# coecms/xmhw

Hardware: AMD Instinct MI355X
Metric: grid-cells/sec for threshold() on 40yr daily SST (higher is better)
Workload: dtype f32 in / f64 out; 1 GPU; 0.25deg global (configs[2]): 1036800 cells per step, 1982-2021 (T=14610), windowHalfWidth=5, pctile=90, smoothPercentileWidth=31, nan_frac=0.0, skipna=False; cells_rank0=1036800, T=14610, D=366, kernel=clim_sorted_f32 (sorted row-lists in LDS, 2 lanes per cell, layout 40), slabs=1, gather=none

## Files before the change

xmhw_amd/csrc/capi.cpp:

```cpp
#include "../../include/xmhw_amd.h"

#include <hip/hip_runtime.h>
#include <unistd.h>

#include <cerrno>

#include <algorithm>
#include <cstdio>
#include <cstdlib>
#include <atomic>
#include <cstring>
#include <map>
#include <memory>
#include <mutex>
#include <new>
#include <string>
#include <type_traits>
#include <vector>

#include "kernels.h"
#include "plan.h"

namespace {

// ... 1081 lines not shown
    const int32_t y2 = v2 >= 0 ? xmhw::ring2_pick_yps(plan->host.w, plan->host.ntracks, v2) : 0;
    *layout = (ring && y2 > 0 && xmhw::ring2_f32_supported(plan->host.w, y2, v2)) ? v2 : -1;
    return XMHW_OK;
}
int xmhw_plan_set_ring2(xmhw_plan* plan, int32_t variant) { return xmhw_plan_set_layout(plan, variant); }
int xmhw_plan_ring2_in_use(const xmhw_plan* plan, int32_t* variant) { return xmhw_plan_layout_in_use(plan, variant); }
int xmhw_plan_f64_mode(const xmhw_plan* plan, int32_t* variant) {
    if (!plan || !variant) return fail(XMHW_ERR_INVALID, "NULL argument");
    *variant = resolve_kernel(plan, 8) == XMHW_KERNEL_RING ? x64_choice(plan).variant : -1;
    return XMHW_OK;
}
int xmhw_plan_destroy(xmhw_plan* plan) {
    delete plan;
    return XMHW_OK;
}
int xmhw_plan_info(const xmhw_plan* plan, int32_t* D, int32_t* ntracks, int32_t* kernel, int32_t* nsteps,
                   int32_t* step_min) {
    if (!plan) return fail(XMHW_ERR_INVALID, "plan is NULL");
    if (D) *D = plan->host.D;
    if (ntracks) *ntracks = plan->host.ntracks;
    if (kernel) *kernel = resolve_kernel(plan, 4);
    if (nsteps) *nsteps = plan->host.nsteps;
    if (step_min) *step_min = plan->host.step_min;
    return XMHW_OK;
}
int xmhw_plan_doys(const xmhw_plan* plan, int32_t* doys_out) {
    if (!plan || !doys_out) return fail(XMHW_ERR_INVALID, "NULL argument");
    std::memcpy(doys_out, plan->host.doys.data(), sizeof(int32_t) * plan->host.doys.size());
    return XMHW_OK;
}
int xmhw_plan_set_kernel(xmhw_plan* plan, int32_t kernel) {
    if (!plan) return fail(XMHW_ERR_INVALID, "plan is NULL");
    if (kernel < XMHW_KERNEL_AUTO || kernel > XMHW_KERNEL_GENERIC)
        return fail(XMHW_ERR_INVALID, "unknown kernel selector");
    plan->host.kernel_choice = kernel;
    return XMHW_OK;
}
int xmhw_plan_set_timing(xmhw_plan* plan, int32_t enable) {
    if (!plan) return fail(XMHW_ERR_INVALID, "plan is NULL");
    plan->timing = enable != 0;
    return XMHW_OK;
}
int xmhw_plan_kernel_ms(xmhw_plan* plan, int32_t calls_back, float* ms) {
    if (!plan || !ms) return fail(XMHW_ERR_INVALID, "NULL argument");
    if (calls_back < 0 || calls_back >= 16 || static_cast<uint64_t>(calls_back) >= plan->tcalls)
        return fail(XMHW_ERR_INVALID, "no such timed call");
    const int slot = static_cast<int>((plan->tcalls - 1 - static_cast<uint64_t>(calls_back)) % 16);
    if (!plan->tev[2 * slot] || !plan->tev[2 * slot + 1]) return fail(XMHW_ERR_INVALID, "no such timed call");
    HIP_TRY(hipEventSynchronize(plan->tev[2 * slot + 1]));
    HIP_TRY(hipEventElapsedTime(ms, plan->tev[2 * slot], plan->tev[2 * slot + 1]));
    return XMHW_OK;
}
int xmhw_plan_set_narrowing(xmhw_plan* plan, int32_t enable) {
    if (!plan) return fail(XMHW_ERR_INVALID, "plan is NULL");
    plan->narrowing = enable != 0;
    return XMHW_OK;
}
int xmhw_plan_narrowed(xmhw_plan* plan, int32_t* narrowed_out) {
    if (!plan || !narrowed_out) return fail(XMHW_ERR_INVALID, "NULL argument");
    *narrowed_out = 0;
    if (!plan->d_narrow_flag) return XMHW_OK;
    uint32_t flag = 1;
    HIP_TRY(hipMemcpy(&flag, plan->d_narrow_flag, sizeof(uint32_t), hipMemcpyDeviceToHost));
    *narrowed_out = flag == 0 ? 1 : 0;
    return XMHW_OK;
}
int xmhw_plan_set_chunks(xmhw_plan* plan, int32_t nchunks) {
    if (!plan) return fail(XMHW_ERR_INVALID, "plan is NULL");
    if (nchunks < 0) return fail(XMHW_ERR_INVALID, "nchunks must be >= 0");
    plan->host.nchunks_req = nchunks;
    return XMHW_OK;
}
int xmhw_plan_chunks_in_use(const xmhw_plan* plan, int64_t C, int32_t* nchunks) {
    if (!plan || !nchunks) return fail(XMHW_ERR_INVALID, "NULL argument");
    if (C < 0) return fail(XMHW_ERR_INVALID, "bad C");
    *nchunks = auto_chunks(plan, std::max<int64_t>(C, 1));
    return XMHW_OK;
}
int xmhw_debug_stats_available(void) { return xmhw::ring_stats_built() ? 1 : 0; }
int xmhw_plan_debug_stats_n(xmhw_plan* plan, int enable, uint64_t* out, int32_t n) {
    if (!plan) return fail(XMHW_ERR_INVALID, "plan is NULL");
    if (out && n <= 0) return fail(XMHW_ERR_INVALID, "n must be > 0");
    if (enable && !plan->d_stats) {
        HIP_TRY(hipMalloc(&plan->d_stats, 16 * sizeof(unsigned long long)));
        HIP_TRY(hipMemset(plan->d_stats, 0, 16 * sizeof(unsigned long long)));
    }
    if (out) {
        if (!plan->d_stats) return fail(XMHW_ERR_INVALID, "stats not enabled");
        unsigned long long all[16];
        HIP_TRY(hipDeviceSynchronize());
        HIP_TRY(hipMemcpy(all, plan->d_stats, sizeof(all), hipMemcpyDeviceToHost));
        HIP_TRY(hipMemset(plan->d_stats, 0, sizeof(all)));
        for (int32_t i = 0; i < std::min<int32_t>(n, 16); ++i) out[i] = all[i];
    }
    return XMHW_OK;
}
int xmhw_plan_debug_stats(xmhw_plan* plan, int enable, uint64_t* out8) {
    return xmhw_plan_debug_stats_n(plan, enable, out8, 8);
}
int xmhw_plan_table(const xmhw_plan* plan, int32_t years_per_lane, uint32_t* table_out,
                    int32_t* ntracks_padded) {
    if (!plan) return fail(XMHW_ERR_INVALID, "plan is NULL");
    if (years_per_lane <= 0) return fail(XMHW_ERR_INVALID, "years_per_lane must be > 0");
    if (plan->host.ntracks > kSubs * years_per_lane)
        return fail(XMHW_ERR_INVALID, "years_per_lane too small for the number of tracks");
    if (ntracks_padded) *ntracks_padded = kSubs * years_per_lane;
    if (table_out) {
        std::vector<uint32_t> tab = plan->host.ring_table(kSubs, years_per_lane);
        std::memcpy(table_out, tab.data(), sizeof(uint32_t) * tab.size());
    }
    return XMHW_OK;
}

int xmhw_plan_sorted_info(const xmhw_plan* plan, int64_t C, int32_t* keys_per_list, int32_t* lds_bytes_per_wave,
                          int32_t* pieces) {
    if (!plan) return fail(XMHW_ERR_INVALID, "plan is NULL");
    const int32_t k = xmhw::sorted_pick_k(plan->host.w, plan->host.ntracks);
    if (k == 0) return fail(XMHW_ERR_UNSUPPORTED, "the sorted-list kernel is not instantiated for this window / record length");
    if (keys_per_list) *keys_per_list = k;
    if (lds_bytes_per_wave) *lds_bytes_per_wave = xmhw::sorted_lds_bytes(plan->host.w, plan->host.ntracks);
    if (pieces) {
        const int64_t waves = (std::max<int64_t>(C, 1) + 31) / 32;
        *pieces = static_cast<int32_t>(plan->host.nchunks_req > 0 ? plan->host.nchunks_req : (1536 + waves - 1) / waves);
    }
    return XMHW_OK;
}

int xmhw_plan_sorted_table(const xmhw_plan* plan, int32_t pieces, int32_t* nchunks, int32_t* nrows, int32_t* ntp,
                           int32_t* chunks_out, uint32_t* table_out, uint32_t* flags_out) {
    if (!plan) return fail(XMHW_ERR_INVALID, "plan is NULL");
    const int32_t yps = xmhw::sorted_pick_yps(plan->host.w, plan->host.ntracks);
    if (yps == 0) return fail(XMHW_ERR_UNSUPPORTED, "the sorted-list kernel is not instantiated for this window / record length");
    const xmhw::Plan::SortedPlan sp = plan->host.sorted_plan(2 * yps, 24, std::max(pieces, 1));
    if (nchunks) *nchunks = static_cast<int32_t>(sp.chunks.size());
    if (nrows) *nrows = static_cast<int32_t>(sp.flags.size());
    if (ntp) *ntp = 2 * yps;
    if (chunks_out)
        for (size_t i = 0; i < sp.chunks.size(); ++i) {
            chunks_out[4 * i + 0] = sp.chunks[i].warm_start;
            chunks_out[4 * i + 1] = sp.chunks[i].begin;
            chunks_out[4 * i + 2] = sp.chunks[i].end;
            chunks_out[4 * i + 3] = sp.chunks[i].trow0;
        }
    if (table_out) std::memcpy(table_out, sp.table.data(), sizeof(uint32_t) * sp.table.size());
    if (flags_out) std::memcpy(flags_out, sp.flags.data(), sizeof(uint32_t) * sp.flags.size());
    return XMHW_OK;
}

int xmhw_clim_raw_f32(xmhw_plan* plan, const float* ts, int64_t C, int64_t ld, double q, int negate,
                      double* thresh, double* seas, int64_t ldo, void* stream) {
    return clim_raw<float>(plan, ts, C, ld, q, negate, thresh, seas, ldo, stream);
}
int xmhw_clim_raw_f64(xmhw_plan* plan, const double* ts, int64_t C, int64_t ld, double q, int negate,
                      double* thresh, double* seas, int64_t ldo, void* stream) {
    return clim_raw<double>(plan, ts, C, ld, q, negate, thresh, seas, ldo, stream);
}

int xmhw_clim_raw_i16(xmhw_plan* plan, const int16_t* codes, int64_t C, int64_t ld, int big_endian, int has_scale,
                      double scale_factor, double add_offset, int has_fill, int32_t fill_code, int decoded_itemsize, double q,
                      int negate, double* thresh, double* seas, int64_t ldo, void* stream) {
    if (!plan) return fail(XMHW_ERR_INVALID, "plan is NULL");
    if (C < 0 || ld < C || ldo < C) return fail(XMHW_ERR_INVALID, "bad C/ld/ldo");
    if (!(q >= 0.0 && q <= 1.0)) return fail(XMHW_ERR_INVALID, "quantile must be in [0, 1]");
    if (decoded_itemsize != 4 && decoded_itemsize != 8) return fail(XMHW_ERR_INVALID, "decoded_itemsize must be 4 or 8");
    if (has_scale && !(scale_factor == scale_factor && add_offset == add_offset && scale_factor != 0.0))
        return fail(XMHW_ERR_INVALID, "scale_factor must be a non-zero number, add_offset a number");
    if (C == 0) return XMHW_OK;
    if (!codes || !thresh || !seas) return fail(XMHW_ERR_INVALID, "NULL device buffer");
    int rc = upload(plan, C);
    if (rc != XMHW_OK) return rc;
    if (!(plan->nchunks_s > 0 && sorted_serves(q)))
        return fail(XMHW_ERR_UNSUPPORTED, "packed input runs on the sorted-list kernel only (w = 5, 9..48 tracks, quantile >= 0.85 or <= 0.15): "
                                         "decode the series (xmhw_decode) and call xmhw_clim_raw_f32 / _f64");
    xmhw::PackedI16 pk;
    pk.swap = big_endian ? 1 : 0;
    pk.fill = has_fill ? fill_code : 0x7FFFFFFF;
// ... 301 lines not shown
```

xmhw_amd/csrc/kernels_sorted.hip:

```cpp
#include <type_traits>

#include "device_common.h"
#include "kernels.h"
#include "packed_src.h"
#include "plan.h"
#include "sortnet_gen.h"

namespace xmhw {
namespace {

typedef __attribute__((address_space(3))) uint32_t lds_u32;
__device__ __forceinline__ uint32_t lds_ld(uint32_t a) { return *reinterpret_cast<lds_u32*>(static_cast<uintptr_t>(a)); }
__device__ __forceinline__ void lds_st(uint32_t a, uint32_t v) { *reinterpret_cast<lds_u32*>(static_cast<uintptr_t>(a)) = v; }

constexpr int kSwap1 = 0xB1;
__device__ __forceinline__ uint32_t swp(uint32_t v) {
    return static_cast<uint32_t>(__builtin_amdgcn_update_dpp(0, static_cast<int>(v), kSwap1, 0xF, 0xF, true));
}
__device__ __forceinline__ double swp(double v) {
    const uint64_t b = static_cast<uint64_t>(__double_as_longlong(v));
    const uint32_t lo = swp(static_cast<uint32_t>(b)), hi = swp(static_cast<uint32_t>(b >> 32));
    return __longlong_as_double(static_cast<long long>((static_cast<uint64_t>(hi) << 32) | lo));
}
__device__ __forceinline__ uint32_t med3u(uint32_t a, uint32_t b, uint32_t c) {
// ... 197 lines not shown
    const char* col = static_cast<const char*>(ts) + (cell_ok ? cell : C - 1) * static_cast<int64_t>(ES);
    const bool mirror = q < 0.5;
    const int kneg = (negate != 0) != mirror ? 1 : 0;
    const uint32_t tmax = static_cast<uint32_t>(Tn - 1);
    const bool padded_last = (YPS - 1) * 2 + sub >= ntracks;
    const uint32_t padmask = padded_last ? 0xFFFFFFFFu : 0u;
    const uint32_t* tab = table + sub;

    const uint32_t lds0 = static_cast<uint32_t>(reinterpret_cast<uintptr_t>((lds_u32*)lds));
    if (lds0 != 0u) __builtin_trap();
    const uint32_t lcell = static_cast<uint32_t>(cw) * 4u;
    for (int i = lane; i < LDS_BYTES / 4; i += 64) lds[i] = 0u;
    __builtin_amdgcn_s_waitcnt(0);
    __builtin_amdgcn_wave_barrier();

    uint32_t P[NL];
    V32 TV = 0;
#define XMHW_RSLO(j) TV[2 * (j)]
#define XMHW_RSHI(j) TV[2 * (j) + 1]
#define XMHW_EX(e, j) TV[12 + 6 * (e) + (j)]
#define XMHW_NVL(j) TV[24 + (j)]
    uint32_t lbase[NL];
#pragma unroll
    for (int j = 0; j < NL; ++j) {
        const int g = sub * NL + j;
        lbase[j] = g < R ? lcell + static_cast<uint32_t>(g) * LSTRIDE : 0x40000000u + lcell;
        P[j] = 0;
    }
    static_assert(KL >= 5, "a list holds a window");
    static_assert(NL == 6 && EXT <= 2, "the register vector holds five values of six lists");
#ifdef XMHW_WARM_SELECT
    uint32_t Ctop = 0, n = 0, B = 0u;
#else
    uint32_t Ctop = 0, n = 0, B = 0xFFFFFFFFu;
#endif
    double total = 0.0;

    const uint32_t ld4 = static_cast<uint32_t>(ld) * ES;
    const char* ap[YPS];
    auto entries_of = [&](int32_t step, uint32_t (&e)[YPS]) {
        const uint32_t* p = tab + static_cast<int64_t>(step - step_min) * NTP;
#pragma unroll
        for (int y = 0; y < YPS; ++y) e[y] = p[y * 2];
    };
    auto point_at = [&](int32_t step) {
        uint32_t e[YPS];
        entries_of(step, e);
#pragma unroll
        for (int y = 0; y < YPS; ++y) {
            const uint32_t t = umin((e[y] >> 1) - 2u, tmax);
            ap[y] = col + static_cast<uint64_t>(t) * ld4;
        }
    };
    auto advance = [&]() {
#pragma unroll
        for (int y = 0; y < YPS; ++y) ap[y] += (y == YPS - 1 && padded_last) ? 0u : ld4;
    };
    typename std::conditional<PACKED, int32_t, float>::type x_in[YPS];
    auto request = [&]() {
#pragma unroll
        for (int y = 0; y < YPS; ++y) {
            if constexpr (PACKED) x_in[y] = static_cast<int32_t>(*reinterpret_cast<const int16_t*>(ap[y]));
            else x_in[y] = *reinterpret_cast<const float*>(ap[y]);
        }
    };
    point_at(ch.warm_start);
    request();

    unsigned long long tacc[8] = {0, 0, 0, 0, 0, 0, 0, 0};
    unsigned long long tlast = 0;
    if constexpr (STATS) tlast = __builtin_amdgcn_s_memtime();
    auto tick = [&](int idx) {
        if constexpr (STATS) {
            __builtin_amdgcn_sched_barrier(0);
            asm volatile("s_waitcnt lgkmcnt(0)" ::: "memory");
            const unsigned long long now = __builtin_amdgcn_s_memtime();
            tacc[idx] += now - tlast;
            tlast = now;
            __builtin_amdgcn_sched_barrier(0);
        }
    };
    uint32_t st_rows = 0, st_iter = 0, st_flag = 0, st_steps = 0;
    uint32_t st_serial = 0, st_ext = 0;
    uint32_t st_more[4] = {0, 0, 0, 0};

    uint32_t e_alo = 0, e_ahi = 0, e_n = 0;
    double e_total = 0.0, e_g = 0.0;

    int32_t ep_s = -1;
    uint32_t ep_eph = 0;
    auto finish_rows = [&]() {
        double th = make_nan(), se = make_nan();
        if (e_n > 0) {
            double v_lo = static_cast<double>(key_f32(e_alo));
            double v_hi = static_cast<double>(key_f32(e_ahi));
            if (mirror) {
                v_lo = -v_lo;
                v_hi = -v_hi;
            }
            se = e_total / static_cast<double>(e_n);
            if constexpr (PACKED) {
                v_lo = packed_value(pk, v_lo);
                v_hi = packed_value(pk, v_hi);
                se = packed_value(pk, se);
            }
            th = numpy_lerp(v_lo, v_hi, e_g);
        }
        if (static_cast<uint32_t>(sub) <= ep_eph && cell_ok) {
            const int64_t row = static_cast<int64_t>(ep_s) - static_cast<int64_t>(ep_eph) + sub;
            thresh[row * ldo + cell] = th;
            seas[row * ldo + cell] = se;
        }
        ep_s = -1;
    };
    bool nan_mode = false;
    uint32_t vi_n = 0xFFFFFFFFu, vi_lo = 0;
    double vi_g = 0.0;
    int m = ((ch.warm_start % R) + R) % R;
    uint32_t sf_cur = __builtin_amdgcn_readfirstlane(sflags[ch.warm_start - step_min]);
    uint32_t sf_nxt = ch.warm_start + 1 < ch.end ? __builtin_amdgcn_readfirstlane(sflags[ch.warm_start + 1 - step_min]) : 0u;
#ifdef XMHW_LOOP_ALIGN
    asm volatile(".p2align " XMHW_STR(XMHW_LOOP_ALIGN) "\n\t.rept " XMHW_STR(XMHW_LOOP_PAD) "\n\ts_nop 0\n\t.endr" ::: "memory");
#endif
    for (int32_t s = ch.warm_start; s < ch.end; ++s) {
        const uint32_t sf = sf_cur;
        const uint32_t sf_nn = s + 2 < ch.end ? sflags[s + 2 - step_min] : 0u;
        uint32_t k[HE];
        double din = 0.0;
        uint32_t nvin = 0;
        float xv[YPS];
        bool packed_fill = false;
        if constexpr (STATS) {
            asm volatile("s_waitcnt vmcnt(0)" ::: "memory");
            tick(5);
        }
        if constexpr (PACKED) {
            if (pk.swap) {
#pragma unroll
                for (int y = 0; y < YPS; ++y)
                    x_in[y] = static_cast<int32_t>(static_cast<int16_t>(__builtin_bswap16(static_cast<uint16_t>(x_in[y]))));
            }
#pragma unroll
            for (int y = 0; y < YPS; ++y) xv[y] = static_cast<float>(x_in[y]);
            if (pk.mode == 1) {
#pragma unroll
                for (int y = 0; y < YPS; ++y) {
                    float f = xv[y] * pk.sf;
                    f = f + pk.of;
                    xv[y] = f;
                }
            }
            bool anyfill = false;
#pragma unroll
            for (int y = 0; y < YPS; ++y) anyfill = anyfill || x_in[y] == pk.fill;
            packed_fill = wave_any(anyfill);
            if (packed_fill) {
#pragma unroll
                for (int y = 0; y < YPS; ++y) xv[y] = x_in[y] == pk.fill ? __uint_as_float(0x7FC00000u) : xv[y];
            }
        } else {
#pragma unroll
            for (int y = 0; y < YPS; ++y) xv[y] = x_in[y];
        }
        bool slow = !(sf & 1u) || nan_mode;
        if (!slow) {
            auto plain_row = [&](auto negc, auto sumc) {
// ... 439 lines not shown
                    pv[j] = sat ? c_ : 0u;
                    need += pv[j];
                }
                need += swp(need);
                if constexpr (STATS) ++st_ext;
                const bool fix = need != 0u;
                auto heads = [&](uint32_t (&hd)[NL]) -> uint32_t {
                    uint32_t lv[NL];
#pragma unroll
                    for (int j = 0; j < NL; ++j) lv[j] = lds_ld(lbase[j] + (P[j] - 1u) * RSTRIDE);
                    uint32_t hm = 0xFFFFFFFFu;
#pragma unroll
                    for (int j = 0; j < NL; ++j) {
                        uint32_t ev = XMHW_EX(0, j);
#pragma unroll
                        for (int e_ = 1; e_ < EXT; ++e_) ev = pv[j] > static_cast<uint32_t>(e_) ? XMHW_EX(e_, j) : ev;
                        hd[j] = (pv[j] != 0u ? ev : lv[j]) - 1u;
                        hm = umin(hm, hd[j]);
                    }
                    return hm;
                };
                uint32_t vlast = a_lo;
                while (wave_any(need != 0u)) {
                    uint32_t hd[NL];
                    const uint32_t hm = heads(hd);
                    const uint32_t ho = swp(hm);
                    const uint32_t cmin = umin(hm, ho);
                    const bool act = need != 0u;
                    const bool win = act && hm == cmin && (sub == 0 || ho != cmin);
                    bool found = false;
#pragma unroll
                    for (int j = 0; j < NL; ++j) {
                        const bool sel = win && !found && hd[j] == cmin;
                        const bool reg = pv[j] != 0u;
                        P[j] = (sel && !reg) ? P[j] - 1u : P[j];
                        pv[j] = (sel && reg) ? pv[j] - 1u : pv[j];
                        found = found || sel;
                    }
                    if (act) {
                        vlast = cmin + 1u;
                        need -= 1u;
                    }
                }
                uint32_t hd[NL];
                uint32_t hm = heads(hd);
                hm = umin(hm, swp(hm)) + 1u;
                uint32_t pvs = 0;
#pragma unroll
                for (int j = 0; j < NL; ++j) pvs += pv[j];
                pvs += swp(pvs);
                if (fix) {
                    a_lo = vlast;
                    a_hi = hm;
                    if (!need2) {
                        if (mirror) a_lo = a_hi;
                        else a_hi = a_lo;
                    }
                    Ctop = Cs - pvs;
#pragma unroll
                    for (int j = 0; j < NL; ++j) flag = flag || (pv[j] == static_cast<uint32_t>(EXT) && XMHW_NVL(j) > static_cast<uint32_t>(K));
                }
            }
        } else {
            uint32_t atb = 0;
#pragma unroll
            for (int j = 0; j < NL; ++j)
                atb |= (P[j] == static_cast<uint32_t>(K) && XMHW_NVL(j) > static_cast<uint32_t>(K)) ? (1u << j) : 0u;
            if (XMHW_COLD(wave_any(atb != 0u))) {
#pragma unroll
                for (int j = 0; j < NL; ++j) {
                    const uint32_t Uj = lds_ld(lbase[j] + static_cast<uint32_t>(K - 1) * RSTRIDE);
                    flag = flag || (((atb >> j) & 1u) && Uj > a_lo);
                }
            }
        }
        B = a_lo;
        {
            const uint32_t fl_ = flag ? 1u : 0u;
            flag = (fl_ | swp(fl_)) != 0u;
        }
        if constexpr (STATS) st_flag += (sub == 0 && cell_ok && flag) ? 1u : 0u;
        tick(3);
        if (XMHW_COLD(s >= ch.begin && wave_any(flag))) {
            constexpr int KPL = (NTP * R + 63) / 64;
            unsigned long long fm = __builtin_amdgcn_ballot_w64(flag && sub == 0 && cell_ok);
            while (fm != 0ull) {
                const int L = __builtin_ctzll(fm);
                fm &= fm - 1ull;
                const int64_t cc = static_cast<int64_t>(blockIdx.x) * 32 + (L >> 1);
                const uint32_t n_c = static_cast<uint32_t>(__builtin_amdgcn_readlane(static_cast<int>(n), L));
                uint32_t lo_c = static_cast<uint32_t>(__builtin_amdgcn_readlane(static_cast<int>(lo), L));
                if (mirror) lo_c = lo_c + 1u < n_c ? n_c - 2u - lo_c : 0u;
                const uint32_t guess = static_cast<uint32_t>(__builtin_amdgcn_readlane(static_cast<int>(a_lo), L));
                uint32_t key[KPL];
                {
                    uint32_t ent[KPL];
#pragma unroll
                    for (int i = 0; i < KPL; ++i) {
                        const int e = lane + 64 * i;
                        const int j = e / NTP, trk = e - j * NTP;
                        ent[i] = e < NTP * R ? table[static_cast<int64_t>(s - j - step_min) * NTP + trk] : (kCodeInvalid << 1);
                    }
                    const char* colc = static_cast<const char*>(ts) + cc * static_cast<int64_t>(ES);
                    typename std::conditional<PACKED, int32_t, float>::type raw[KPL];
#pragma unroll
                    for (int i = 0; i < KPL; ++i) {
                        const uint32_t t = umin((ent[i] >> 1) - 2u, tmax);
                        const char* a_ = colc + static_cast<uint64_t>(t) * ld4;
                        if constexpr (PACKED) raw[i] = static_cast<int32_t>(*reinterpret_cast<const int16_t*>(a_));
                        else raw[i] = *reinterpret_cast<const float*>(a_);
                    }
#pragma unroll
                    for (int i = 0; i < KPL; ++i) {
                        float xs;
                        if constexpr (PACKED) {
                            int32_t c_ = raw[i];
                            if (pk.swap) c_ = static_cast<int32_t>(static_cast<int16_t>(__builtin_bswap16(static_cast<uint16_t>(c_))));
                            xs = packed_sample(pk, c_);
                        } else {
                            xs = raw[i];
                        }
                        const bool ok = xs == xs && (ent[i] >> 1) >= 2u;
                        const uint32_t kk = kneg ? key_fast<true>(__float_as_uint(xs)) : key_fast<false>(__float_as_uint(xs));
                        key[i] = ok ? kk : 0u;
                    }
                }
                uint32_t r_lo = 0, r_hi = 0;
                pool_order_stats<KPL>(key, n_c, lo_c, guess, r_lo, r_hi);
                const bool mine = (lane >> 1) == (L >> 1);
                if (mirror && !(lo_c + 1u < n_c && n_c >= 2u)) r_hi = r_lo;
                a_lo = mine ? r_lo : a_lo;
                a_hi = mine ? r_hi : a_hi;
                flag = mine ? false : flag;
            }
        }
        tick(7);
        if constexpr (STATS) st_steps += (sub == 0 && cell_ok) ? steps0 : 0u;
        }
        tick(3);

        if (s >= ch.begin) {
            if constexpr (STATS) ++st_rows;
            const uint32_t eph = static_cast<uint32_t>(s - ch.begin) & 1u;
            if (static_cast<uint32_t>(sub) == eph) {
                e_alo = mirror ? a_hi : a_lo;
                e_ahi = mirror ? a_lo : a_hi;
                e_n = n;
                e_total = total;
                e_g = g;
            }
            if (eph == 1u || s + 1 == ch.end) {
                ep_s = s;
                ep_eph = eph;
            }
        }
        tick(4);
        sf_cur = sf_nxt;
        sf_nxt = __builtin_amdgcn_readfirstlane(sf_nn);
    }
    if (ep_s >= 0) finish_rows();
    if (STATS && stats != nullptr) {
        if (lane == 0) {
            atomicAdd(&stats[0], static_cast<unsigned long long>(st_rows));
            atomicAdd(&stats[1], static_cast<unsigned long long>(st_iter));
#pragma unroll
            for (int i = 1; i < 4; ++i) atomicAdd(&stats[4 + i], static_cast<unsigned long long>(st_more[i]));
            atomicAdd(&stats[4], static_cast<unsigned long long>(st_ext));
#pragma unroll
            for (int i = 0; i < 8; ++i) atomicAdd(&stats[8 + i], tacc[i]);
        }
        if (sub == 0) {
            atomicAdd(&stats[2], static_cast<unsigned long long>(st_flag));
            atomicAdd(&stats[3], static_cast<unsigned long long>(st_steps));
        }
    }
}

#ifndef XMHW_WAVES3_MAX_YPS
#define XMHW_WAVES3_MAX_YPS 8
#endif
#define XMHW_WAVES_PER_SIMD(Y) ((Y) <= XMHW_WAVES3_MAX_YPS ? 3 : 2)
template <int YPS, int K, int KL, bool STATS>
__global__ __launch_bounds__(64, XMHW_WAVES_PER_SIMD(YPS)) void clim_sorted_f32(
    const float* __restrict__ ts, int64_t C, int64_t ld, int64_t Tn, const uint32_t* __restrict__ table,
    const uint32_t* __restrict__ sflags, const DevSortedChunk* __restrict__ chunks, double q, int negate,
    int32_t ntracks, double* __restrict__ thresh, double* __restrict__ seas, int64_t ldo,
    unsigned long long* __restrict__ stats) {
    sorted_body<YPS, K, KL, STATS, false>(ts, C, ld, Tn, table, sflags, chunks, q, negate, ntracks, thresh, seas, ldo, stats,
                                      PackedI16{});
}
template <int YPS, int K, int KL>
__global__ __launch_bounds__(64, XMHW_WAVES_PER_SIMD(YPS)) void clim_sorted_i16(
    const int16_t* __restrict__ codes, PackedI16 pk, int64_t C, int64_t ld, int64_t Tn, const uint32_t* __restrict__ table,
    const uint32_t* __restrict__ sflags, const DevSortedChunk* __restrict__ chunks, double q, int negate,
    int32_t ntracks, double* __restrict__ thresh, double* __restrict__ seas, int64_t ldo) {
    sorted_body<YPS, K, KL, false, true>(codes, C, ld, Tn, table, sflags, chunks, q, negate, ntracks, thresh, seas, ldo, nullptr, pk);
}

namespace {
typedef void (*SortedKernel)(const float*, int64_t, int64_t, int64_t, const uint32_t*, const uint32_t*,
                             const DevSortedChunk*, double, int, int32_t, double*, double*, int64_t, unsigned long long*);
typedef void (*SortedKernelI16)(const int16_t*, PackedI16, int64_t, int64_t, int64_t, const uint32_t*, const uint32_t*,
                                const DevSortedChunk*, double, int, int32_t, double*, double*, int64_t);
struct SortedEntry { int yps, k, kl; SortedKernel fn, fn_stats; SortedKernelI16 fn_i16; };
#ifdef XMHW_RING_STATS
#define XMHW_SS(Y, K, KL) clim_sorted_f32<Y, K, KL, true>
#else
#define XMHW_SS(Y, K, KL) nullptr
#endif
#define XMHW_S2(Y, K, KL) {Y, K, KL, clim_sorted_f32<Y, K, KL, false>, XMHW_SS(Y, K, KL), clim_sorted_i16<Y, K, KL>}
#define XMHW_S(Y, K) XMHW_S2(Y, K, K)
#ifndef XMHW_K40
#define XMHW_K40 16
#endif
#ifndef XMHW_KL48
#define XMHW_KL48 16
#endif
#ifndef XMHW_KL40
#define XMHW_KL40 14
#endif
const SortedEntry kSorted[] = {
#ifdef XMHW_SORTED_ONLY
    XMHW_S2(20, XMHW_K40, XMHW_KL40),
#else
    XMHW_S(5, 6),   XMHW_S(6, 6),   XMHW_S(7, 8),   XMHW_S(8, 8),   XMHW_S(9, 10),  XMHW_S(10, 10), XMHW_S(11, 10),
    XMHW_S(12, 10), XMHW_S(13, 12), XMHW_S(14, 12), XMHW_S(15, 12), XMHW_S(16, 12), XMHW_S(17, 14), XMHW_S(18, 14),
    XMHW_S2(19, XMHW_K40, XMHW_KL40), XMHW_S2(20, XMHW_K40, XMHW_KL40), XMHW_S2(21, 18, XMHW_KL48), XMHW_S2(22, 18, XMHW_KL48), XMHW_S2(23, 18, XMHW_KL48), XMHW_S2(24, 18, XMHW_KL48),
#endif
};
#undef XMHW_S
#undef XMHW_S2
#undef XMHW_SS
const SortedEntry* find_sorted(int32_t yps) {
    for (const auto& e : kSorted)
        if (e.yps == yps) return &e;
    return nullptr;
}
}

namespace {
__global__ __launch_bounds__(64) void lds_outside_probe(uint32_t* __restrict__ bad, int BYTES) {
    extern __shared__ __attribute__((aligned(16))) uint32_t lds[];
    for (int i = threadIdx.x; i < BYTES / 4; i += 64) lds[i] = 0x80000000u | (blockIdx.x << 16) | static_cast<uint32_t>(i);
    __builtin_amdgcn_s_waitcnt(0);
    __builtin_amdgcn_wave_barrier();
    const uint32_t base = static_cast<uint32_t>(reinterpret_cast<uintptr_t>((lds_u32*)lds));
    uint32_t wrong = base != 0u ? 1u : 0u;
    const uint32_t lane4 = threadIdx.x * 4u;
    constexpr uint32_t RS = 11u * 128u;
    for (uint32_t r = 0; r < 6; ++r) {
// ... 68 lines not shown
```

xmhw_amd/csrc/pybind.cpp:

```cpp
#include <pybind11/numpy.h>
#include <algorithm>
#include <pybind11/pybind11.h>

#include <cstdint>
#include <stdexcept>
#include <string>

#include "../../include/xmhw_amd.h"

namespace py = pybind11;

namespace {

struct HipError : std::runtime_error { using std::runtime_error::runtime_error; };
struct InvalidError : std::runtime_error { using std::runtime_error::runtime_error; };
struct CommError : std::runtime_error { using std::runtime_error::runtime_error; };

void check(int rc) {
    if (rc == XMHW_OK) return;
    std::string msg = xmhw_last_error();
    if (rc == XMHW_ERR_INVALID) throw InvalidError(msg);
    if (rc == XMHW_ERR_NOMEM) throw std::bad_alloc();
    if (rc == XMHW_ERR_COMM) throw CommError(msg);
    throw HipError(msg + " (code " + std::to_string(rc) + ")");
// ... 43 lines not shown
        py::buffer_info bi = src.request();
        if (bi.ndim != 2 || bi.strides[1] != bi.itemsize || bi.strides[0] < bi.itemsize * bi.shape[1])
            throw InvalidError("memcpy2d_h2d needs a 2-D array with contiguous rows");
        if (col0 < 0 || ncols < 0 || col0 + ncols > bi.shape[1]) throw InvalidError("column range outside the array");
        const size_t isz = static_cast<size_t>(bi.itemsize);
        const size_t spitch = static_cast<size_t>(bi.strides[0]);
        py::gil_scoped_release r;
        check(xmhw_memcpy2d_h2d(vp(dst), isz * static_cast<size_t>(ncols), static_cast<const char*>(bi.ptr) + isz * col0,
                                spitch, isz * static_cast<size_t>(ncols), static_cast<size_t>(bi.shape[0]), vp(stream)));
    }, py::arg("dst"), py::arg("src"), py::arg("col0"), py::arg("ncols"), py::arg("stream") = 0);
    m.def("memcpy_d2h", [](py::buffer dst, uintptr_t src, uintptr_t stream) {
        py::buffer_info bi = dst.request(true);
        py::gil_scoped_release r;
        check(xmhw_memcpy_d2h(bi.ptr, vp(src), static_cast<size_t>(bi.size) * bi.itemsize, vp(stream)));
    }, py::arg("dst"), py::arg("src"), py::arg("stream") = 0);
    m.def("memcpy_d2h_bytes", [](py::buffer dst, uintptr_t src, size_t nbytes, uintptr_t stream) {
        py::buffer_info bi = dst.request(true);
        if (nbytes > static_cast<size_t>(bi.size) * bi.itemsize) throw InvalidError("destination too small");
        check(xmhw_memcpy_d2h(bi.ptr, vp(src), nbytes, vp(stream)));
    }, py::arg("dst"), py::arg("src"), py::arg("nbytes"), py::arg("stream") = 0);
    m.def("memset", [](uintptr_t dst, int v, size_t n, uintptr_t stream) { check(xmhw_memset(vp(dst), v, n, vp(stream))); },
          py::arg("dst"), py::arg("value"), py::arg("nbytes"), py::arg("stream") = 0);
    m.def("stream_create", []() { void* s = nullptr; check(xmhw_stream_create(&s)); return reinterpret_cast<uintptr_t>(s); });
    m.def("stream_destroy", [](uintptr_t s) { check(xmhw_stream_destroy(vp(s))); });
    m.def("stream_sync", [](uintptr_t s) { py::gil_scoped_release r; check(xmhw_stream_sync(vp(s))); }, py::arg("stream") = 0);
    m.def("event_create", []() { void* e = nullptr; check(xmhw_event_create(&e)); return reinterpret_cast<uintptr_t>(e); });
    m.def("event_destroy", [](uintptr_t e) { check(xmhw_event_destroy(vp(e))); });
    m.def("event_record", [](uintptr_t e, uintptr_t s) { check(xmhw_event_record(vp(e), vp(s))); }, py::arg("event"), py::arg("stream") = 0);
    m.def("stream_wait_event", [](uintptr_t s, uintptr_t e) { check(xmhw_stream_wait_event(vp(s), vp(e))); });
    m.def("event_elapsed_ms", [](uintptr_t a, uintptr_t b) { float ms = 0; check(xmhw_event_elapsed_ms(vp(a), vp(b), &ms)); return ms; });

    m.def("plan_create", [](i32arr doy, int w) {
        xmhw_plan* p = nullptr;
        check(xmhw_plan_create(doy.data(), doy.size(), w, &p));
        return reinterpret_cast<uintptr_t>(p);
    });
    m.def("plan_destroy", [](uintptr_t p) { check(xmhw_plan_destroy(pp(p))); });
    m.def("plan_info", [](uintptr_t p) {
        int32_t D, nt, k, ns, smin;
        check(xmhw_plan_info(pp(p), &D, &nt, &k, &ns, &smin));
        py::dict r;
        r["D"] = D; r["ntracks"] = nt; r["kernel"] = k; r["nsteps"] = ns; r["step_min"] = smin;
        return r;
    });
    m.def("plan_doys", [](uintptr_t p) {
        int32_t D;
        check(xmhw_plan_info(pp(p), &D, nullptr, nullptr, nullptr, nullptr));
        py::array_t<int32_t> out(D);
        check(xmhw_plan_doys(pp(p), out.mutable_data()));
        return out;
    });
    m.def("plan_set_kernel", [](uintptr_t p, int k) { check(xmhw_plan_set_kernel(pp(p), k)); });
    m.def("plan_set_narrowing", [](uintptr_t p, int on) { check(xmhw_plan_set_narrowing(pp(p), on)); });
    m.def("plan_narrowed", [](uintptr_t p) { int32_t n = 0; check(xmhw_plan_narrowed(pp(p), &n)); return n != 0; });
    m.def("plan_set_chunks", [](uintptr_t p, int n) { check(xmhw_plan_set_chunks(pp(p), n)); });
    m.def("plan_table", [](uintptr_t p, int yps) {
        int32_t ns, ntp;
        check(xmhw_plan_info(pp(p), nullptr, nullptr, nullptr, &ns, nullptr));
        check(xmhw_plan_table(pp(p), yps, nullptr, &ntp));
        py::array_t<uint32_t> out({static_cast<py::ssize_t>(ns), static_cast<py::ssize_t>(ntp)});
        check(xmhw_plan_table(pp(p), yps, out.mutable_data(), &ntp));
        return out;
    });

    m.def("plan_set_timing", [](uintptr_t p, int on) { check(xmhw_plan_set_timing(pp(p), on)); });
    m.def("plan_kernel_ms", [](uintptr_t p, int back) { float ms = 0; check(xmhw_plan_kernel_ms(pp(p), back, &ms)); return ms; });
    m.def("plan_sorted_info", [](uintptr_t p, int64_t C) {
        int32_t k = 0, lds = 0, pieces = 0;
        check(xmhw_plan_sorted_info(pp(p), C, &k, &lds, &pieces));
        return py::make_tuple(k, lds, pieces);
    });
    m.def("plan_sorted_table", [](uintptr_t p, int pieces) {
        int32_t nc = 0, nr = 0, ntp = 0;
        check(xmhw_plan_sorted_table(pp(p), pieces, &nc, &nr, &ntp, nullptr, nullptr, nullptr));
        py::array_t<int32_t> chunks({static_cast<py::ssize_t>(nc), static_cast<py::ssize_t>(4)});
        py::array_t<uint32_t> table({static_cast<py::ssize_t>(nr), static_cast<py::ssize_t>(ntp)});
        py::array_t<uint32_t> flags(static_cast<py::ssize_t>(nr));
        check(xmhw_plan_sorted_table(pp(p), pieces, &nc, &nr, &ntp, chunks.mutable_data(), table.mutable_data(),
                                     flags.mutable_data()));
        return py::make_tuple(chunks, table, flags);
    });

    m.def("plan_debug_stats", [](uintptr_t p, int enable, bool read) {
        py::array_t<uint64_t> out(16);
        std::fill(out.mutable_data(), out.mutable_data() + 16, uint64_t(0));
        check(xmhw_plan_debug_stats_n(pp(p), enable, read ? out.mutable_data() : nullptr, 16));
        return out;
    });
    m.def("plan_chunks_in_use", [](uintptr_t p, int64_t C) { int32_t v = 0; check(xmhw_plan_chunks_in_use(pp(p), C, &v)); return v; });
    m.def("debug_stats_available", []() { return xmhw_debug_stats_available() != 0; });
    m.def("plan_set_layout", [](uintptr_t p, int layout) { check(xmhw_plan_set_layout(pp(p), layout)); });
    m.def("plan_layout_in_use", [](uintptr_t p) { int32_t v = -1; check(xmhw_plan_layout_in_use(pp(p), &v)); return v; });
    m.def("sorted_device_ok", []() { int32_t v = 0; check(xmhw_sorted_device_ok(&v)); return v != 0; });
    m.def("plan_ring2_in_use", [](uintptr_t p) { int32_t v = -1; check(xmhw_plan_ring2_in_use(pp(p), &v)); return v; });
    m.def("plan_f64_mode", [](uintptr_t p) { int32_t v = -1; check(xmhw_plan_f64_mode(pp(p), &v)); return v; });
    m.def("plan_set_ring2", [](uintptr_t p, int variant) { check(xmhw_plan_set_ring2(pp(p), variant)); });

    m.def("clim_raw", [](uintptr_t plan, uintptr_t ts, int itemsize, int64_t C, int64_t ld, double q, int negate,
                         uintptr_t th, uintptr_t se, int64_t ldo, uintptr_t stream) {
        if (itemsize == 4)
            check(xmhw_clim_raw_f32(pp(plan), static_cast<const float*>(vp(ts)), C, ld, q, negate,
                                    static_cast<double*>(vp(th)), static_cast<double*>(vp(se)), ldo, vp(stream)));
        else if (itemsize == 8)
            check(xmhw_clim_raw_f64(pp(plan), static_cast<const double*>(vp(ts)), C, ld, q, negate,
                                    static_cast<double*>(vp(th)), static_cast<double*>(vp(se)), ldo, vp(stream)));
        else throw InvalidError("itemsize must be 4 or 8");
    }, py::arg("plan"), py::arg("ts"), py::arg("itemsize"), py::arg("C"), py::arg("ld"), py::arg("q"),
       py::arg("negate"), py::arg("thresh"), py::arg("seas"), py::arg("ldo"), py::arg("stream") = 0);

    m.def("clim_raw_i16", [](uintptr_t plan, uintptr_t codes, int64_t C, int64_t ld, int big_endian, int has_scale,
                             double scale_factor, double add_offset, int has_fill, int32_t fill_code, int decoded_itemsize,
                             double q, int negate, uintptr_t th, uintptr_t se, int64_t ldo, uintptr_t stream) {
        check(xmhw_clim_raw_i16(pp(plan), static_cast<const int16_t*>(vp(codes)), C, ld, big_endian, has_scale, scale_factor,
                                add_offset, has_fill, fill_code, decoded_itemsize, q, negate, static_cast<double*>(vp(th)),
                                static_cast<double*>(vp(se)), ldo, vp(stream)));
    }, py::arg("plan"), py::arg("codes"), py::arg("C"), py::arg("ld"), py::arg("big_endian"), py::arg("has_scale"),
       py::arg("scale_factor"), py::arg("add_offset"), py::arg("has_fill"), py::arg("fill_code"), py::arg("decoded_itemsize"),
       py::arg("q"), py::arg("negate"), py::arg("thresh"), py::arg("seas"), py::arg("ldo"), py::arg("stream") = 0);

    m.def("clim_finish", [](uintptr_t plan, uintptr_t th_in, uintptr_t se_in, int64_t C, int64_t ldo, int feb29_fix,
                            int smooth, int width, uintptr_t th_out, uintptr_t se_out, uintptr_t stream) {
        check(xmhw_clim_finish(pp(plan), static_cast<const double*>(vp(th_in)), static_cast<const double*>(vp(se_in)),
                               C, ldo, feb29_fix, smooth, width, static_cast<double*>(vp(th_out)),
                               static_cast<double*>(vp(se_out)), vp(stream)));
    }, py::arg("plan"), py::arg("thresh_in"), py::arg("seas_in"), py::arg("C"), py::arg("ldo"),
       py::arg("feb29_fix"), py::arg("smooth"), py::arg("width"), py::arg("thresh_out"), py::arg("seas_out"),
       py::arg("stream") = 0);

    m.def("clim_dev", [](uintptr_t ts, int itemsize, i32arr doy, int64_t C, int D, int w, double q, int smooth,
                         int smooth_w, int feb29_fix, int negate, uintptr_t th, uintptr_t se, uintptr_t stream) {
        py::gil_scoped_release r;
        if (itemsize == 4)
            check(xmhw_clim_f32(static_cast<const float*>(vp(ts)), doy.data(), doy.size(), C, D, w, q, smooth, smooth_w,
                                feb29_fix, negate, static_cast<double*>(vp(th)), static_cast<double*>(vp(se)), vp(stream)));
        else if (itemsize == 8)
            check(xmhw_clim_f64(static_cast<const double*>(vp(ts)), doy.data(), doy.size(), C, D, w, q, smooth, smooth_w,
                                feb29_fix, negate, static_cast<double*>(vp(th)), static_cast<double*>(vp(se)), vp(stream)));
        else throw InvalidError("itemsize must be 4 or 8");
    });

    m.def("clim_host", [](py::array ts, i32arr doy, int D, int w, double q, int smooth, int smooth_w, int feb29_fix,
                          int negate) {
        if (ts.ndim() != 2) throw InvalidError("ts must be (T, C)");
        if (!(ts.flags() & py::array::c_style)) throw InvalidError("ts must be C-contiguous");
        if (ts.shape(0) != doy.size()) throw InvalidError("doy length must equal T");
        const int64_t T = ts.shape(0), C = ts.shape(1);
        py::array_t<double> th({static_cast<py::ssize_t>(D), static_cast<py::ssize_t>(C)});
        py::array_t<double> se({static_cast<py::ssize_t>(D), static_cast<py::ssize_t>(C)});
        int rc;
        if (ts.dtype().is(py::dtype::of<float>())) {
            py::gil_scoped_release r;
            rc = xmhw_clim_host_f32(static_cast<const float*>(ts.data()), doy.data(), T, C, D, w, q, smooth, smooth_w,
                                    feb29_fix, negate, th.mutable_data(), se.mutable_data());
        } else if (ts.dtype().is(py::dtype::of<double>())) {
            py::gil_scoped_release r;
            rc = xmhw_clim_host_f64(static_cast<const double*>(ts.data()), doy.data(), T, C, D, w, q, smooth, smooth_w,
                                    feb29_fix, negate, th.mutable_data(), se.mutable_data());
        } else {
            throw InvalidError("ts dtype must be float32 or float64");
        }
        check(rc);
        return py::make_tuple(th, se);
    });

    m.def("land_mask", [](uintptr_t ts, int itemsize, int64_t T, int64_t C, int64_t ld, int anynans, uintptr_t keep,
                          uintptr_t stream) {
        if (itemsize == 4)
            check(xmhw_land_mask_f32(static_cast<const float*>(vp(ts)), T, C, ld, anynans, static_cast<uint8_t*>(vp(keep)), vp(stream)));
        else if (itemsize == 8)
// ... 306 lines not shown
```

Before: 42.52 million cells/s.

## Resolve flagged cells from LDS rows plus few reloaded short rows before full gather

```diff
diff --git a/xmhw_amd/csrc/capi.cpp b/xmhw_amd/csrc/capi.cpp
--- a/xmhw_amd/csrc/capi.cpp
+++ b/xmhw_amd/csrc/capi.cpp
@@ -1187,16 +1187,16 @@
     if (!plan) return fail(XMHW_ERR_INVALID, "plan is NULL");
     if (out && n <= 0) return fail(XMHW_ERR_INVALID, "n must be > 0");
     if (enable && !plan->d_stats) {
-        HIP_TRY(hipMalloc(&plan->d_stats, 16 * sizeof(unsigned long long)));
-        HIP_TRY(hipMemset(plan->d_stats, 0, 16 * sizeof(unsigned long long)));
+        HIP_TRY(hipMalloc(&plan->d_stats, 32 * sizeof(unsigned long long)));
+        HIP_TRY(hipMemset(plan->d_stats, 0, 32 * sizeof(unsigned long long)));
     }
     if (out) {
         if (!plan->d_stats) return fail(XMHW_ERR_INVALID, "stats not enabled");
-        unsigned long long all[16];
+        unsigned long long all[32];
         HIP_TRY(hipDeviceSynchronize());
         HIP_TRY(hipMemcpy(all, plan->d_stats, sizeof(all), hipMemcpyDeviceToHost));
         HIP_TRY(hipMemset(plan->d_stats, 0, sizeof(all)));
-        for (int32_t i = 0; i < std::min<int32_t>(n, 16); ++i) out[i] = all[i];
+        for (int32_t i = 0; i < std::min<int32_t>(n, 32); ++i) out[i] = all[i];
     }
     return XMHW_OK;
 }
diff --git a/xmhw_amd/csrc/kernels_sorted.hip b/xmhw_amd/csrc/kernels_sorted.hip
--- a/xmhw_amd/csrc/kernels_sorted.hip
+++ b/xmhw_amd/csrc/kernels_sorted.hip
@@ -303,6 +303,7 @@
     };
     uint32_t st_rows = 0, st_iter = 0, st_flag = 0, st_steps = 0;
     uint32_t st_serial = 0, st_ext = 0;
+    uint32_t st_virt = 0, st_full = 0;
     uint32_t st_more[4] = {0, 0, 0, 0};
 
     uint32_t e_alo = 0, e_ahi = 0, e_n = 0;
@@ -908,7 +909,33 @@
         if constexpr (STATS) st_flag += (sub == 0 && cell_ok && flag) ? 1u : 0u;
         tick(3);
         if (XMHW_COLD(s >= ch.begin && wave_any(flag))) {
-            constexpr int KPL = (NTP * R + 63) / 64;
+            constexpr int VL = (R * KL + 63) / 64;
+            constexpr int VX = EXT > 0 ? 1 : 0;
+            constexpr int SMAX = 3;
+            constexpr int VK = VL + VX + SMAX;
+            constexpr bool VIRT = YPS > 8;
+            static_assert(NTP <= 64 && R * EXT <= 64, "a row, and the register ranks, fit a wave");
+            using Raw = typename std::conditional<PACKED, int32_t, float>::type;
+            const uint32_t m_s = static_cast<uint32_t>(((s % R) + R) % R);
+            auto load_at = [&](const char* colc, uint32_t en) -> Raw {
+                const uint32_t t = umin((en >> 1) - 2u, tmax);
+                const char* a_ = colc + static_cast<uint64_t>(t) * ld4;
+                if constexpr (PACKED) return static_cast<int32_t>(*reinterpret_cast<const int16_t*>(a_));
+                else return *reinterpret_cast<const float*>(a_);
+            };
+            auto key_of = [&](Raw r_, uint32_t en) -> uint32_t {
+                float xs;
+                if constexpr (PACKED) {
+                    int32_t c_ = r_;
+                    if (pk.swap) c_ = static_cast<int32_t>(static_cast<int16_t>(__builtin_bswap16(static_cast<uint16_t>(c_))));
+                    xs = packed_sample(pk, c_);
+                } else {
+                    xs = r_;
+                }
+                const bool ok = xs == xs && (en >> 1) >= 2u;
+                const uint32_t kk = kneg ? key_fast<true>(__float_as_uint(xs)) : key_fast<false>(__float_as_uint(xs));
+                return ok ? kk : 0u;
+            };
             unsigned long long fm = __builtin_amdgcn_ballot_w64(flag && sub == 0 && cell_ok);
             while (fm != 0ull) {
                 const int L = __builtin_ctzll(fm);
@@ -918,42 +945,93 @@
                 uint32_t lo_c = static_cast<uint32_t>(__builtin_amdgcn_readlane(static_cast<int>(lo), L));
                 if (mirror) lo_c = lo_c + 1u < n_c ? n_c - 2u - lo_c : 0u;
                 const uint32_t guess = static_cast<uint32_t>(__builtin_amdgcn_readlane(static_cast<int>(a_lo), L));
-                uint32_t key[KPL];
-                {
+                const char* colc = static_cast<const char*>(ts) + cc * static_cast<int64_t>(ES);
+                const uint32_t lc = static_cast<uint32_t>(L >> 1) * 4u;
+                int lane_;
+                asm volatile("v_mbcnt_lo_u32_b32 %0, -1, 0\n\tv_mbcnt_hi_u32_b32 %0, -1, %0" : "=v"(lane_));
+                const int tl_ = lane_ < NTP ? lane_ : 0;
+                uint32_t r_lo = 0, r_hi = 0;
+                bool done = false;
+                if constexpr (VIRT) {
+                    uint32_t sm = 0, mx = 0, xk = 0;
+#pragma unroll
+                    for (int g = 0; g < R; ++g) {
+                        const int jj = g % NL, ln = L + g / NL;
+                        const uint32_t nvl = static_cast<uint32_t>(__builtin_amdgcn_readlane(static_cast<int>(XMHW_NVL(jj)), ln));
+                        uint32_t ex[EXN];
+#pragma unroll
+                        for (int e_ = 0; e_ < EXT; ++e_)
+                            ex[e_] = static_cast<uint32_t>(__builtin_amdgcn_readlane(static_cast<int>(XMHW_EX(e_, jj)), ln));
+                        uint32_t U;
+                        if constexpr (EXT > 0) U = ex[EXT - 1];
+                        else U = static_cast<uint32_t>(__builtin_amdgcn_readfirstlane(static_cast<int>(
+                                lds_ld(lc + static_cast<uint32_t>(g) * LSTRIDE + static_cast<uint32_t>(K - 1) * RSTRIDE))));
+                        const bool hides = nvl > static_cast<uint32_t>(K);
+                        const bool shrt = hides && U >= guess;
+                        sm |= shrt ? (1u << g) : 0u;
+                        mx = (hides && !shrt) ? umax(mx, U) : mx;
+#pragma unroll
+                        for (int e_ = 0; e_ < EXT; ++e_) xk = (lane_ == g + R * e_ && !shrt) ? ex[e_] : xk;
+                    }
+                    if (__builtin_popcount(sm) <= SMAX) {
+                        uint32_t re[SMAX];
+                        Raw rw[SMAX];
+                        uint32_t rest = sm;
+#pragma unroll
+                        for (int k_ = 0; k_ < SMAX; ++k_) {
+                            const uint32_t g = rest != 0u ? static_cast<uint32_t>(__builtin_ctz(rest)) : m_s;
+                            const int32_t j = static_cast<int32_t>((m_s + R - g) % R);
+                            const uint32_t e_ = table[static_cast<int64_t>(s - j - step_min) * NTP + tl_];
+                            re[k_] = rest != 0u && lane_ < NTP ? e_ : (kCodeInvalid << 1);
+                            rest &= rest - 1u;
+                        }
+#pragma unroll
+                        for (int k_ = 0; k_ < SMAX; ++k_) rw[k_] = load_at(colc, re[k_]);
+                        uint32_t vk[VK];
+#pragma unroll
+                        for (int i = 0; i < VL; ++i) {
+                            const uint32_t e = static_cast<uint32_t>(lane_ + 64 * i);
+                            const bool in = e < static_cast<uint32_t>(R * KL) && !((sm >> (e % R)) & 1u);
+                            const uint32_t v_ = lds_ld(lc + (in ? e : 0u) * LSTRIDE);
+                            vk[i] = in ? v_ : 0u;
+                        }
+                        if constexpr (VX > 0) vk[VL] = xk;
+#pragma unroll
+                        for (int k_ = 0; k_ < SMAX; ++k_) vk[VL + VX + k_] = key_of(rw[k_], re[k_]);
+                        uint32_t nv = 0;
+#pragma unroll
+                        for (int i = 0; i < VK; ++i) nv += static_cast<uint32_t>(__builtin_popcountll(__builtin_amdgcn_ballot_w64(vk[i] != 0u)));
+                        const uint32_t h = n_c - nv;
+                        if (nv != 0u && h <= lo_c) {
+                            pool_order_stats<VK>(vk, nv, lo_c - h, guess, r_lo, r_hi);
+                            done = r_lo > mx;
+                        }
+                    }
+                }
+                if constexpr (STATS) {
+                    st_virt += done ? 1u : 0u;
+                    st_full += done ? 0u : 1u;
+                }
+                if (!done) {
+                    constexpr int KPL = (NTP * R + 63) / 64;
                     uint32_t ent[KPL];
 #pragma unroll
                     for (int i = 0; i < KPL; ++i) {
-                        const int e = lane + 64 * i;
-                        const int j = e / NTP, trk = e - j * NTP;
-                        ent[i] = e < NTP * R ? table[static_cast<int64_t>(s - j - step_min) * NTP + trk] : (kCodeInvalid << 1);
+                        const int e = lane_ + 64 * i;
+                        const bool in = e < NTP * R;
+                        const int j = in ? e / NTP : 0, trk = in ? e - j * NTP : 0;
+                        const uint32_t e_ = table[static_cast<int64_t>(s - j - step_min) * NTP + trk];
+                        ent[i] = in ? e_ : (kCodeInvalid << 1);
                     }
-                    const char* colc = static_cast<const char*>(ts) + cc * static_cast<int64_t>(ES);
-                    typename std::conditional<PACKED, int32_t, float>::type raw[KPL];
-#pragma unroll
-                    for (int i = 0; i < KPL; ++i) {
-                        const uint32_t t = umin((ent[i] >> 1) - 2u, tmax);
-                        const char* a_ = colc + static_cast<uint64_t>(t) * ld4;
-                        if constexpr (PACKED) raw[i] = static_cast<int32_t>(*reinterpret_cast<const int16_t*>(a_));
-                        else raw[i] = *reinterpret_cast<const float*>(a_);
-                    }
-#pragma unroll
-                    for (int i = 0; i < KPL; ++i) {
-                        float xs;
-                        if constexpr (PACKED) {
-                            int32_t c_ = raw[i];
-                            if (pk.swap) c_ = static_cast<int32_t>(static_cast<int16_t>(__builtin_bswap16(static_cast<uint16_t>(c_))));
-                            xs = packed_sample(pk, c_);
-                        } else {
-                            xs = raw[i];
-                        }
-                        const bool ok = xs == xs && (ent[i] >> 1) >= 2u;
-                        const uint32_t kk = kneg ? key_fast<true>(__float_as_uint(xs)) : key_fast<false>(__float_as_uint(xs));
-                        key[i] = ok ? kk : 0u;
-                    }
-                }
-                uint32_t r_lo = 0, r_hi = 0;
-                pool_order_stats<KPL>(key, n_c, lo_c, guess, r_lo, r_hi);
-                const bool mine = (lane >> 1) == (L >> 1);
+                    Raw raw[KPL];
+#pragma unroll
+                    for (int i = 0; i < KPL; ++i) raw[i] = load_at(colc, ent[i]);
+                    uint32_t key[KPL];
+#pragma unroll
+                    for (int i = 0; i < KPL; ++i) key[i] = key_of(raw[i], ent[i]);
+                    pool_order_stats<KPL>(key, n_c, lo_c, guess, r_lo, r_hi);
+                }
+                const bool mine = (lane_ >> 1) == (L >> 1);
                 if (mirror && !(lo_c + 1u < n_c && n_c >= 2u)) r_hi = r_lo;
                 a_lo = mine ? r_lo : a_lo;
                 a_hi = mine ? r_hi : a_hi;
@@ -992,6 +1070,8 @@
 #pragma unroll
             for (int i = 1; i < 4; ++i) atomicAdd(&stats[4 + i], static_cast<unsigned long long>(st_more[i]));
             atomicAdd(&stats[4], static_cast<unsigned long long>(st_ext));
+            atomicAdd(&stats[16], static_cast<unsigned long long>(st_virt));
+            atomicAdd(&stats[17], static_cast<unsigned long long>(st_full));
 #pragma unroll
             for (int i = 0; i < 8; ++i) atomicAdd(&stats[8 + i], tacc[i]);
         }
diff --git a/xmhw_amd/csrc/pybind.cpp b/xmhw_amd/csrc/pybind.cpp
--- a/xmhw_amd/csrc/pybind.cpp
+++ b/xmhw_amd/csrc/pybind.cpp
@@ -149,9 +149,9 @@
     });
 
     m.def("plan_debug_stats", [](uintptr_t p, int enable, bool read) {
-        py::array_t<uint64_t> out(16);
-        std::fill(out.mutable_data(), out.mutable_data() + 16, uint64_t(0));
-        check(xmhw_plan_debug_stats_n(pp(p), enable, read ? out.mutable_data() : nullptr, 16));
+        py::array_t<uint64_t> out(32);
+        std::fill(out.mutable_data(), out.mutable_data() + 32, uint64_t(0));
+        check(xmhw_plan_debug_stats_n(pp(p), enable, read ? out.mutable_data() : nullptr, 32));
         return out;
     });
     m.def("plan_chunks_in_use", [](uintptr_t p, int64_t C) { int32_t v = 0; check(xmhw_plan_chunks_in_use(pp(p), C, &v)); return v; });
```

New measurement: 43.04 million cells/s, median of 6. 1.2% higher.
